# nzw0301/SimCLR

Hardware: AMD Instinct MI355X
Metric: pretrain images/sec (whole node) + CIFAR-10 linear-probe top-1, ResNet-50 (higher is better)
Workload: dtype bf16

## Files before the change

### simclr_amd/csrc/bindings.cpp

```cpp
#include <ATen/core/Tensor.h>
#include <ATen/ops/empty.h>
#include <ATen/ops/zeros.h>
#include <ATen/hip/HIPContext.h>
#include <c10/util/Exception.h>
#include <torch/library.h>

#include <algorithm>
#include <vector>

#include "kernels.h"

using at::Tensor;

namespace {

hipStream_t cur_stream() { return at::hip::getCurrentHIPStream().stream(); }

void check_dev(const Tensor& t, at::ScalarType dt, const char* name) {
  TORCH_CHECK(t.is_cuda(), name, ": expected a GPU tensor");
  TORCH_CHECK(t.scalar_type() == dt, name, ": expected dtype ", dt, " got ", t.scalar_type());
  TORCH_CHECK(t.is_contiguous(), name, ": expected a contiguous tensor");
}

const uint16_t* bf(const Tensor& t, const char* n) {
// ... 176 lines not shown
  if (f.pro_sc) {
    TORCH_CHECK(pro_seg_rows > 0 && pro_seg_rows % bm == 0 && M % pro_seg_rows == 0,
                "igemm prologue: segment rows must be a multiple of the tile rows");
    TORCH_CHECK(pro_sc->numel() >= (M / pro_seg_rows) * g.C, "igemm prologue: [S][C] size");
  }
  if (pro_d.has_value() && pro_d->defined()) {
    TORCH_CHECK(f.pro_sc, "igemm BN-backward prologue needs pro_sc (A) and pro_sh (B)");
    TORCH_CHECK(pro_d->numel() >= (M / pro_seg_rows) * g.C, "igemm prologue: d [S][C] size");
    TORCH_CHECK(A2.has_value() && A2->numel() == A.numel(), "igemm prologue: A2 must match A");
    TORCH_CHECK(epi_mode == 0 || epi_mode == 3 || epi_mode == 4,
                "igemm BN-backward prologue: epilogue 0, 3 or 4");
    TORCH_CHECK(!(igemm_variant_patch((int)variant) && epi_mode == 4),
                "igemm BN-backward prologue on a patch variant: epilogue 0 or 3");
    f.pro_d = f32(*pro_d, "pro_d");
    f.A2 = bf(*A2, "A2");
    if (pro_out.has_value() && pro_out->defined()) {
      TORCH_CHECK(igemm_variant_patch((int)variant) && (epi_mode == 0 || epi_mode == 3),
                  "igemm: the materialised BN-backward operand (pro_out) needs a patch variant "
                  "and epilogue 0 or 3");
      TORCH_CHECK(pro_out->numel() == A.numel(), "igemm: pro_out must match A");
      const char* o0 = static_cast<const char*>(pro_out->data_ptr());
      const char* o1 = o0 + pro_out->numel() * 2;
      for (const Tensor* t : {&A, &*A2, &out}) {
        const char* t0 = static_cast<const char*>(t->data_ptr());
        const char* t1 = t0 + t->numel() * t->element_size();
        TORCH_CHECK(!(o0 < t1 && t0 < o1), "igemm: pro_out must not alias A, A2 or out");
      }
      f.pro_out = bfw(*pro_out, "pro_out");
    }
  }
  if (dual) {
    TORCH_CHECK(f.pro_sc && f.pro_sh && !f.pro_d && epi_mode == 0 && !(bias.has_value() && bias->defined()),
                "igemm block-output prologue: scale/shift tables, no other fusion");
    TORCH_CHECK(A2.has_value() && A2->numel() == A.numel(), "igemm block-output prologue: residual");
    TORCH_CHECK(pro_out->numel() == A.numel(), "igemm block-output prologue: out size");
    TORCH_CHECK(pro_mask.has_value() && pro_mask->defined() && pro_mask->numel() * 8 >= A.numel(),
                "igemm block-output prologue: mask size");
    check_dev(*pro_mask, at::kByte, "pro_mask");
    TORCH_CHECK(pro_relu, "igemm block-output prologue: always applies ReLU (pro_relu required)");
    auto overlaps = [](const Tensor& a, const Tensor& b) {
      const char* a0 = static_cast<const char*>(a.data_ptr());
      const char* b0 = static_cast<const char*>(b.data_ptr());
      const char* a1 = a0 + a.numel() * a.element_size();
      const char* b1 = b0 + b.numel() * b.element_size();
      return a0 < b1 && b0 < a1;
    };
    TORCH_CHECK(!overlaps(*pro_out, A) && !overlaps(*pro_out, *A2) && !overlaps(*pro_out, out) &&
                    !overlaps(*pro_mask, A) && !overlaps(*pro_mask, *A2) && !overlaps(*pro_mask, out),
                "igemm block-output prologue: out / mask must not alias A, the residual or the "
                "conv output");
    f.A2 = bf(*A2, "A2");
    f.pro_out = bfw(*pro_out, "pro_out");
    f.pro_mask = pro_mask->data_ptr<uint8_t>();
    if (pro_rss.has_value() && pro_rss->defined()) {
      const int64_t nseg = M / pro_seg_rows;
      TORCH_CHECK(pro_rss->numel() >= 2 * nseg * g.C, "igemm block-output prologue: rss [2][S][C]");
      f.pro_rsc = f32(*pro_rss, "pro_rss");
      f.pro_rsh = f.pro_rsc + nseg * g.C;
    }
  }
  conv_igemm_nt(g, bf(A, "A"), (size_t)A.numel(), bf(B, "B"), bfw(out, "out"), optf32(bias, "bias"),
                optf32w(stats, "stats"), f, (int)variant, cur_stream());
}

int64_t igemm_bm(int64_t N) { return igemm_block_m((int)N); }
int64_t igemm_nvariants() { return igemm_num_variants(); }
int64_t igemm_vbm(int64_t v) { return igemm_variant_bm((int)v); }
int64_t igemm_vbn(int64_t v) { return igemm_variant_bn((int)v); }
bool igemm_vglds(int64_t v) { return igemm_variant_glds((int)v); }
bool igemm_gldsok(std::vector<int64_t> gv, bool pro, bool bn_bwd_pro) {
  return igemm_glds_ok(geom_from(gv), pro, bn_bwd_pro);
}
int64_t wgrad_nvariants() { return wgrad_num_variants(); }
int64_t wgrad_xlin_op(int64_t mode) { return wgrad_xlin((int)mode); }
bool wgrad_vglds(int64_t v) { return wgrad_variant_glds((int)v); }
bool igemm_vok(int64_t v, std::vector<int64_t> gv, bool pro, bool bnb, int64_t epi_mode) {
  return igemm_variant_ok((int)v, geom_from(gv), pro, bnb, (int)epi_mode);
}
bool igemm_dok(int64_t v, std::vector<int64_t> gv) { return igemm_dual_ok((int)v, geom_from(gv)); }
bool wgrad_vok(int64_t v, std::vector<int64_t> gv, bool pro, bool dpro) {
  return wgrad_variant_ok((int)v, geom_from(gv), pro, dpro);
}

int64_t wgrad_nsplit(std::vector<int64_t> gv, int64_t variant) {
  return wgrad_splits(geom_from(gv), (int)variant);
}

int64_t wgrad_ntiles(std::vector<int64_t> gv, int64_t variant) {
  return wgrad_tiles(geom_from(gv), (int)variant);
}

void wgrad(const Tensor& dY, const Tensor& X, const Tensor& partial, const Tensor& out,
           std::vector<int64_t> gv, int64_t splits, int64_t creal, double beta,
           const c10::optional<Tensor>& pro_sc, const c10::optional<Tensor>& pro_sh,
           int64_t pro_seg_rows, bool pro_relu, int64_t pro_S, int64_t variant,
           const c10::optional<Tensor>& dY2, const c10::optional<Tensor>& dp_coef,
           int64_t dp_seg_rows, int64_t dp_S) {
  const ConvGeom g = geom_from(gv);
  const int64_t M = (int64_t)g.Nb * g.OH * g.OW;
  const int64_t K = (int64_t)g.KH * g.KW * g.C;
  TORCH_CHECK(dY.numel() == M * g.N, "wgrad: dY numel mismatch");
  TORCH_CHECK(X.numel() == (int64_t)g.Nb * g.IH * g.IW * g.C, "wgrad: X numel mismatch");
  TORCH_CHECK(partial.numel() >= splits * g.N * K, "wgrad: partial too small");
  TORCH_CHECK(out.numel() == (int64_t)g.N * g.KH * g.KW * creal, "wgrad: out numel mismatch");
  TORCH_CHECK(creal <= g.C && creal > 0, "wgrad: bad creal");
  TORCH_CHECK(pro_S >= 1 && pro_S <= 2, "wgrad prologue supports at most 2 segments");
  if (variant < 0 || variant >= wgrad_num_variants()) variant = wgrad_default_variant(g.N);
  TORCH_CHECK(wgrad_variant_ok((int)variant, g, pro_sc.has_value() && pro_sc->defined(),
                               dY2.has_value() && dY2->defined()),
              "wgrad: variant ", variant, " is not admissible here: an LDS-DMA variant needs "
              "C % 64 == 0, no dY prologue, and an X prologue only on unpadded 1x1 convolutions "
              "(wgrad_pipe / wgrad_xp: none); the patch variant needs its 3x3 stride-1 geometry, "
              "N % 64 == 0 and no dY prologue");
  ConvFusion f = fusion_from(pro_sc, pro_sh, pro_seg_rows, pro_relu, pro_S, 0, c10::nullopt,
                             c10::nullopt, g.C, 0);
  if (f.pro_sc) {
    TORCH_CHECK(pro_seg_rows > 0 && (int64_t)g.Nb % pro_S == 0, "wgrad prologue geometry");
  }
  if (dY2.has_value() && dY2->defined()) {
    TORCH_CHECK(dY2->numel() == dY.numel(), "wgrad: dY2 must match dY");
    TORCH_CHECK(dp_coef.has_value() && dp_coef->numel() >= 3 * dp_S * g.N, "wgrad: dp_coef [3][S][N]");
    const int64_t iters = (M + 63) / 64;
    const int64_t ips = (iters + splits - 1) / splits;
    TORCH_CHECK(dp_seg_rows > 0 && M % dp_seg_rows == 0 && M / dp_seg_rows == dp_S &&
                    (dp_S <= 2 || dp_seg_rows % (ips * 64) == 0) && dp_seg_rows % 64 == 0,
                "wgrad dY prologue: 64-row segments, and every split inside one segment when "
                "there are more than two");
    f.dY2 = bf(*dY2, "dY2");
    f.dp_coef = f32(*dp_coef, "dp_coef");
    f.dp_seg_rows = (int)dp_seg_rows;
    f.dp_S = (int)dp_S;
  }
  conv_wgrad(g, bf(dY, "dY"), bf(X, "X"), (size_t)X.numel(), f32w(partial, "partial"), (int)splits,
             f32w(out, "out"), (int)creal, (float)beta, f, (int)variant, cur_stream());
}


void conv1x1_bwd_dual_op(const Tensor& G, const c10::optional<Tensor>& A3,
                         const c10::optional<Tensor>& coef, const Tensor& X,
                         const c10::optional<Tensor>& xss, const c10::optional<Tensor>& xmi,
                         const Tensor& Wt, const Tensor& gm,
                         const Tensor& stats, const Tensor& wpart, int64_t S, int64_t bps,
                         const c10::optional<Tensor>& Xraw, bool dual8) {
  const int64_t CI = gm.size(-1);
  const int64_t M = gm.numel() / CI;
  const int64_t CO = G.numel() / M;
  const uint16_t* xr = optbf(Xraw, "Xraw");
  TORCH_CHECK((CO == 256 && CI == 64 && xr == nullptr) || (CO == 512 && CI == 128),
              "conv1x1_bwd_dual: (Co, Ci) = (256, 64) or (512, 128); a pre-applied X (Xraw "
              "given) only with (512, 128)");
  if (xr != nullptr) TORCH_CHECK(Xraw->numel() == M * CI, "conv1x1_bwd_dual: Xraw size");
  TORCH_CHECK(G.numel() == M * CO && X.numel() == M * CI && Wt.numel() == CI * CO,
              "conv1x1_bwd_dual: operand sizes");
  TORCH_CHECK(S >= 1 && S <= 2 && bps >= 1 && M % S == 0 && (M / S) % (64 * bps) == 0,
              "conv1x1_bwd_dual: every block's rows must lie in one segment (64-row tiles)");
  const float* xs = optf32(xss, "xss");
  const float* xm = optf32(xmi, "xmi");
  TORCH_CHECK((xs == nullptr) == (xm == nullptr), "conv1x1_bwd_dual: xss and xmi together");
  TORCH_CHECK(xs != nullptr || (CO == 256 && CI == 64 && xr == nullptr),
              "conv1x1_bwd_dual: the plain form is (Co, Ci) = (256, 64) only");
  if (xs != nullptr) {
    TORCH_CHECK(xss->numel() >= 2 * S * CI && xmi->numel() >= 2 * S * CI,
                "conv1x1_bwd_dual: BN2 tables");
    TORCH_CHECK(stats.numel() >= S * bps * 2 * CI, "conv1x1_bwd_dual: stats size");
  }
  TORCH_CHECK(wpart.numel() >= S * bps * CO * CI, "conv1x1_bwd_dual: wpart size");
  TORCH_CHECK(M * CO * 2 < (int64_t(1) << 31), "conv1x1_bwd_dual: 32-bit buffer offsets");
  const uint16_t* a3 = optbf(A3, "A3");
  const float* cf = optf32(coef, "coef");
  if (a3 != nullptr) {
    TORCH_CHECK(A3->numel() == G.numel() && cf != nullptr && coef->numel() >= 3 * S * CO,
                "conv1x1_bwd_dual: lazy BN-backward needs A3 [M][Co] and coef [3][S][Co]");
  }
  conv1x1_bwd_dual(bf(G, "G"), a3, cf, bf(X, "X"), xs, xm,
                   bf(Wt, "Wt"), bfw(gm, "gm"), f32w(stats, "stats"), f32w(wpart, "wpart"),
                   (int)M, (int)CO, (int)CI, (int)S, (int)bps, cur_stream(), xr, dual8);
}

void conv1x1_bwd_dual_s2_op(const Tensor& G, const c10::optional<Tensor>& A3,
                            const c10::optional<Tensor>& coef, const Tensor& X, const Tensor& Wt,
                            const Tensor& gm, const Tensor& wpart, int64_t S, int64_t bps) {
  TORCH_CHECK(X.dim() == 4 && gm.dim() == 4, "conv1x1_bwd_dual_s2: NHWC 4-D X and gm");
  const int64_t N = X.size(0), H = X.size(1), W = X.size(2), CI = X.size(3);
  const int64_t OH = gm.size(1), OW = gm.size(2);
  TORCH_CHECK(gm.size(0) == N && gm.size(3) == CI && OH == (H + 1) / 2 && OW == (W + 1) / 2,
              "conv1x1_bwd_dual_s2: gm is the stride-2 output map");
  const int64_t Mo = N * OH * OW;
  const int64_t CO = G.numel() / Mo;
  TORCH_CHECK(CO == 512 && CI == 256 && G.numel() == Mo * CO && Wt.numel() == CI * CO,
              "conv1x1_bwd_dual_s2: (Co, Ci) = (512, 256) only");
  TORCH_CHECK(S >= 1 && S <= 2 && N % S == 0 && bps >= 1 && (Mo / S) % (64 * bps) == 0,
              "conv1x1_bwd_dual_s2: every block's rows must lie in one segment");
  TORCH_CHECK(wpart.numel() >= S * bps * CO * CI, "conv1x1_bwd_dual_s2: wpart size");
  TORCH_CHECK(Mo * CO * 2 < (int64_t(1) << 31) && X.numel() * 2 < (int64_t(1) << 31),
              "conv1x1_bwd_dual_s2: 32-bit buffer offsets");
  const uint16_t* a3 = optbf(A3, "A3");
  const float* cf = optf32(coef, "coef");
  TORCH_CHECK(a3 == nullptr && cf == nullptr,
              "conv1x1_bwd_dual_s2: dY must be materialised (no lazy BN-backward form)");
  conv1x1_bwd_dual_s2(bf(G, "G"), a3, cf, bf(X, "X"), bf(Wt, "Wt"), bfw(gm, "gm"),
                      f32w(wpart, "wpart"), (int)Mo, (int)CO, (int)CI, (int)S, (int)bps, (int)H,
                      (int)W, (int)OH, (int)OW, cur_stream());
}

void wgrad_reduce_slabs_op(const Tensor& partial, int64_t splits, const Tensor& out, double beta) {
  const int64_t n = out.numel();
  TORCH_CHECK(n % 4 == 0 && partial.numel() >= splits * n && splits >= 1,
              "wgrad_reduce_slabs: sizes");
  wgrad_reduce_slabs(f32w(partial, "partial"), (int)splits, f32w(out, "out"), (size_t)n,
                     (float)beta, cur_stream());
}

void weight_transform(const Tensor& W, const Tensor& Wt, std::vector<int64_t> p) {
  TORCH_CHECK(p.size() == 10, "weight_transform params");
  const int Co = p[0], KH = p[1], KW = p[2], Ci = p[3], KHs = p[4], KWs = p[5];
  TORCH_CHECK(W.numel() == (int64_t)Co * KH * KW * Ci, "weight_transform: W numel");
  TORCH_CHECK(Wt.numel() == (int64_t)Ci * KHs * KWs * Co, "weight_transform: Wt numel");
  for (int a = 0; a < KHs; ++a) {
    const int kh = (int)p[6] + a * (int)p[7];
    TORCH_CHECK(kh >= 0 && kh < KH, "weight_transform: kh out of range");
  }
  for (int a = 0; a < KWs; ++a) {
    const int kw = (int)p[8] + a * (int)p[9];
    TORCH_CHECK(kw >= 0 && kw < KW, "weight_transform: kw out of range");
  }
  conv_weight_transform(bf(W, "W"), bfw(Wt, "Wt"), Co, KH, KW, Ci, KHs, KWs, p[6], p[7], p[8], p[9],
                        cur_stream());
}

Tensor weight_transform_plan(const std::vector<Tensor>& Ws, const std::vector<Tensor>& Wts,
                             std::vector<int64_t> p) {
  const size_t n = Ws.size();
  TORCH_CHECK(n > 0 && Wts.size() == n && p.size() == 10 * n, "weight_transform_plan sizes");
  Tensor host = at::empty({(int64_t)(n * sizeof(WtDesc) / 8) + 1},
                          at::TensorOptions().dtype(at::kLong));
  WtDesc* d = reinterpret_cast<WtDesc*>(host.data_ptr<int64_t>());
  int blk = 0;
  for (size_t i = 0; i < n; ++i) {
    const int64_t* q = p.data() + 10 * i;
    const int Co = q[0], KH = q[1], KW = q[2], Ci = q[3], KHs = q[4], KWs = q[5];
    TORCH_CHECK(Ws[i].numel() == (int64_t)Co * KH * KW * Ci, "weight_transform_plan: W numel");
    TORCH_CHECK(Wts[i].numel() == (int64_t)Ci * KHs * KWs * Co, "weight_transform_plan: Wt numel");
    TORCH_CHECK(Ws[i].device() == Wts[0].device() && Wts[i].device() == Wts[0].device(),
                "weight_transform_plan: one device");
    for (int a = 0; a < KHs; ++a)
      TORCH_CHECK(q[6] + a * q[7] >= 0 && q[6] + a * q[7] < KH, "weight_transform_plan: kh");
    for (int a = 0; a < KWs; ++a)
      TORCH_CHECK(q[8] + a * q[9] >= 0 && q[8] + a * q[9] < KW, "weight_transform_plan: kw");
    const int nb = ((Co + 63) / 64) * ((Ci + 63) / 64) * KHs * KWs;
    d[i] = WtDesc{bf(Ws[i], "W"), bfw(Wts[i], "Wt"), Co, KH, KW, Ci, KHs, KWs, (int)q[6],
                  (int)q[7], (int)q[8], (int)q[9], blk, nb};
    blk += nb;
  }
  host.data_ptr<int64_t>()[n * sizeof(WtDesc) / 8] = blk;
  return host;
}

void weight_transform_batch(const Tensor& table, int64_t total_blocks) {
  TORCH_CHECK(table.is_cuda() && table.scalar_type() == at::kLong && table.numel() % 8 == 0 &&
                  table.numel() > 0 && total_blocks > 0,
              "weight_transform_batch: device descriptors from weight_transform_plan");
  conv_weight_transform_batch(reinterpret_cast<const WtDesc*>(table.data_ptr<int64_t>()),
                              (int)(table.numel() / 8), (int)total_blocks, cur_stream());
}

void check_rc(const Tensor& x, int64_t S, const char* n) {
  TORCH_CHECK(x.dim() >= 2, n, ": rank");
  const int64_t C = x.size(-1);
  TORCH_CHECK(C % 8 == 0, n, ": channels must be a multiple of 8");
  const int64_t CH = C / 8;
  TORCH_CHECK(CH <= 256 || CH % 256 == 0, n, ": unsupported channel count");
  TORCH_CHECK((x.numel() / C) % S == 0, n, ": rows not divisible by segments");
}

int64_t bn_blocks(int64_t R, int64_t C, int64_t S) {
  return bn_stats_blocks_per_seg((int)R, (int)C, (int)S);
}

void bn_stats(const Tensor& x, int64_t S, const Tensor& partial) {
  check_rc(x, S, "bn_stats");
  const int C = x.size(-1), R = x.numel() / C;
  const int nblk = bn_stats_blocks_per_seg(R, C, S);
  TORCH_CHECK(partial.numel() >= (int64_t)S * nblk * 2 * C, "bn_stats: partial too small");
  bn_stats_partial(bf(x, "x"), R, C, S, f32w(partial, "partial"), nullptr, cur_stream());
}

void bn_reduce(const Tensor& partial, int64_t nblk, int64_t S, int64_t C, const Tensor& stats) {
  TORCH_CHECK(partial.numel() >= S * nblk * 2 * C && stats.numel() >= 2 * S * C, "bn_reduce sizes");
  const int G = bn_reduce_groups((int)nblk);
  TORCH_CHECK(G == 1 || C % 4 == 0, "bn_reduce: C must be a multiple of 4 (float4 partial rows)");
  at::Tensor ws;
  float* wsp = nullptr;
  if (G > 1) {
    ws = at::empty({S * G * 2 * C}, stats.options());
    wsp = ws.data_ptr<float>();
  }
  bn_reduce_partials(f32(partial, "partial"), nblk, S, C, f32w(stats, "stats"), wsp, cur_stream());
}

void bn_final(const Tensor& stats, int64_t S, int64_t C, double count, double eps, double momentum,
              const c10::optional<Tensor>& rm, const c10::optional<Tensor>& rv, const Tensor& mi,
              const c10::optional<Tensor>& nbt, const c10::optional<Tensor>& gamma,
              const c10::optional<Tensor>& beta, const c10::optional<Tensor>& ss) {
  if (ss.has_value() && ss->defined()) TORCH_CHECK(ss->numel() >= 2 * S * C, "bn_finalize: ss size");
  if (gamma.has_value() && gamma->defined()) TORCH_CHECK(gamma->numel() == C, "bn_finalize: gamma");
  if (beta.has_value() && beta->defined()) TORCH_CHECK(beta->numel() == C, "bn_finalize: beta");
  TORCH_CHECK(stats.numel() >= 2 * S * C && mi.numel() >= 2 * S * C, "bn_finalize sizes");
  int64_t* nb = nullptr;
// ... 1073 lines not shown
```

### simclr_amd/csrc/conv.hip

```cpp
#include <cstring>
#include "common.h"
#include "kernels.h"

#include <type_traits>
#include <utility>

namespace {

struct IgemmArgs {
  const uint16_t* A;
  const uint16_t* B;
  uint16_t* out;
  const float* bias;
  float* stats;
  int M, N, K;
  int IH, IW, C;
  int OH, OW, KW;
  int ish, isw, dh, dw, ih0, iw0;
  int OHp, OWp, osh, osw, ooh, oow, ldo;
  int direct_out;
  uint32_t a_bytes, b_bytes;
  int nMb, nNb;
  const float* pro_sc;
  const float* pro_sh;
// ... 2515 lines not shown
#pragma unroll
    for (int j = 0; j < 8; ++j) {
      const uint32_t off = (uint32_t)(((size_t)(m0 + grow + 8 * j) * CO + gch * 8) * 2);
      G8[j] = __builtin_amdgcn_raw_buffer_load_b128(rg, off, 0, 0);
      if (lazy) A8[j] = __builtin_amdgcn_raw_buffer_load_b128(ra, off, 0, 0);
    }
#pragma unroll
    for (int j = 0; j < 2; ++j)
      X2[j] = __builtin_amdgcn_raw_buffer_load_b128(
          rx, (uint32_t)(((size_t)(m0 + xrow + 32 * j) * CI + xch * 8) * 2), 0, 0);
  };
  auto lstore = [&](int buf, const u32x4 (&G8)[8], const u32x4 (&A8)[8], const u32x4 (&X2)[2]) {
#pragma unroll
    for (int j = 0; j < 8; ++j) {
      const int r = grow + 8 * j;
      *(u32x4*)(Ds + buf * BMT * CO + r * CO + tr_swz<CO>(r, gch * 8)) =
          lazy ? bnbwd8(G8[j], A8[j], cA, cB, cD, true) : G8[j];
    }
#pragma unroll
    for (int j = 0; j < 2; ++j) {
      const int r = xrow + 32 * j;
      *(u32x4*)(Xs + buf * BMT * CI + r * CI + tr_swz<CI>(r, xch * 8)) =
          PLAIN ? X2[j] : affine_relu8(X2[j], xsc, xsh, true, true);
      if (!PLAIN) *(u32x4*)(Xr + buf * BMT * CI + r * CI + xch * 8) = X2[j];
    }
  };

  f32x4 accw[4][4];
#pragma unroll
  for (int i = 0; i < 4; ++i)
#pragma unroll
    for (int j = 0; j < 4; ++j) accw[i][j] = (f32x4){0.f, 0.f, 0.f, 0.f};
  float s1[4][4], s2[4][4];
#pragma unroll
  for (int i = 0; i < 4; ++i)
#pragma unroll
    for (int j = 0; j < 4; ++j) { s1[i][j] = 0.f; s2[i][j] = 0.f; }

  auto compute = [&](int t) {
    const int cur = t & 1;
    const uint16_t* Db = Ds + cur * BMT * CO;
    f32x4 accd[4];
#pragma unroll
    for (int fn = 0; fn < 4; ++fn) accd[fn] = (f32x4){0.f, 0.f, 0.f, 0.f};
    const int mrow = wid * 16 + li;
#pragma unroll
    for (int ks = 0; ks < CO / 32; ++ks) {
      const int lch = ks * 4 + g;
      const bf16x8 bfr = *(const bf16x8*)(Db + mrow * CO + tr_swz<CO>(mrow, lch * 8));
#pragma unroll
      for (int fn = 0; fn < 4; ++fn) {
        const int wr = fn * 16 + li;
        const bf16x8 af = *(const bf16x8*)(Ws + wr * CO + ((lch ^ (wr & 7)) * 8));
        accd[fn] = __builtin_amdgcn_mfma_f32_16x16x32_bf16(af, bfr, accd[fn], 0, 0, 0);
      }
    }
    wgrad_mma<CO, CI, 4, 1>(Db, Xs + cur * BMT * CI, accw);
    const int m = mbeg + t * BMT + mrow;
    if constexpr (PLAIN) {
#pragma unroll
      for (int fn = 0; fn < 4; ++fn) {
        const int ci = fn * 16 + 4 * g;
        const u32x2 w = {pack2bf(accd[fn][0], accd[fn][1]), pack2bf(accd[fn][2], accd[fn][3])};
        __builtin_nontemporal_store(w, (u32x2*)(p.gm + (size_t)m * CI + ci));
      }
      return;
    }
    const uint16_t* xr = Xr + cur * BMT * CI + mrow * CI;
#pragma unroll
    for (int fn = 0; fn < 4; ++fn) {
      const int ci = fn * 16 + 4 * g;
      const u32x2 yv = *(const u32x2*)(xr + ci);
      const float4 tsc = *(const float4*)(Tb + ci), tsh = *(const float4*)(Tb + CI + ci);
      const float4 tmu = *(const float4*)(Tb + 2 * CI + ci);
      const float4 tin = *(const float4*)(Tb + 3 * CI + ci);
      const float y[4] = {lo_bf(yv.x), hi_bf(yv.x), lo_bf(yv.y), hi_bf(yv.y)};
      const float sc4[4] = {tsc.x, tsc.y, tsc.z, tsc.w}, sh4[4] = {tsh.x, tsh.y, tsh.z, tsh.w};
      const float mu4[4] = {tmu.x, tmu.y, tmu.z, tmu.w}, in4[4] = {tin.x, tin.y, tin.z, tin.w};
      float gv[4];
#pragma unroll
      for (int r = 0; r < 4; ++r) {
        const float a = bf2f(f2bf(accd[fn][r]));
        gv[r] = y[r] * sc4[r] + sh4[r] > 0.f ? a : 0.f;
        s1[fn][r] += gv[r];
        s2[fn][r] += gv[r] * ((y[r] - mu4[r]) * in4[r]);
      }
      const u32x2 w = {pack2bf(gv[0], gv[1]), pack2bf(gv[2], gv[3])};
      __builtin_nontemporal_store(w, (u32x2*)(p.gm + (size_t)m * CI + ci));
    }
  };

  if (T > 0) {
    gload(0, rG[0], rA[0], rX[0]);
    lstore(0, rG[0], rA[0], rX[0]);
  }
  if (T > 1) gload(1, rG[1], rA[1], rX[1]);
  __syncthreads();
  for (int t = 0; t < T; t += 2) {
    if (t + 2 < T) gload(t + 2, rG[0], rA[0], rX[0]);
    compute(t);
    if (t + 1 < T) lstore(1, rG[1], rA[1], rX[1]);
    asm volatile("s_waitcnt lgkmcnt(0)" ::: "memory");
    __builtin_amdgcn_s_barrier();
    if (t + 1 >= T) break;
    if (t + 3 < T) gload(t + 3, rG[1], rA[1], rX[1]);
    compute(t + 1);
    if (t + 2 < T) lstore(0, rG[0], rA[0], rX[0]);
    asm volatile("s_waitcnt lgkmcnt(0)" ::: "memory");
    __builtin_amdgcn_s_barrier();
  }
  __syncthreads();
  float* wp = p.wpart + (size_t)blk * CO * CI;
#pragma unroll
  for (int fm = 0; fm < 4; ++fm)
#pragma unroll
    for (int fn = 0; fn < 4; ++fn)
#pragma unroll
      for (int i = 0; i < 4; ++i)
        wp[(size_t)(wid * 64 + fm * 16 + g * 4 + i) * CI + fn * 16 + li] = accw[fm][fn][i];
  if (PLAIN) return;
#pragma unroll
  for (int off = 1; off < 16; off <<= 1)
#pragma unroll
    for (int fn = 0; fn < 4; ++fn)
#pragma unroll
      for (int r = 0; r < 4; ++r) {
        s1[fn][r] += __shfl_xor(s1[fn][r], off, 64);
        s2[fn][r] += __shfl_xor(s2[fn][r], off, 64);
      }
  if (li == 0) {
#pragma unroll
    for (int fn = 0; fn < 4; ++fn)
#pragma unroll
      for (int r = 0; r < 4; ++r) {
        const int ci = fn * 16 + 4 * g + r;
        red[(wid * CI + ci) * 2 + 0] = s1[fn][r];
        red[(wid * CI + ci) * 2 + 1] = s2[fn][r];
      }
  }
  __syncthreads();
  if (tid < CI) {
    float a = 0.f, b = 0.f;
#pragma unroll
    for (int w = 0; w < 4; ++w) {
      a += red[(w * CI + tid) * 2 + 0];
      b += red[(w * CI + tid) * 2 + 1];
    }
    p.stats[((size_t)blk * 2 + 0) * CI + tid] = a;
    p.stats[((size_t)blk * 2 + 1) * CI + tid] = b;
  }
}

template <int CO, int CIT, bool LAZY, bool XPRE, bool PLAIN = false, bool XS2 = false,
          int BMT = 32>
__global__ __launch_bounds__(512, 1) void conv1x1_bwd_dual_w(Dual1x1Args p) {
  constexpr int CI = 64;
  constexpr int NH = CIT / CI;
  constexpr int NT = 512;
  constexpr int RG = BMT / 16;
  constexpr int CQ = 8 / RG;
  constexpr int CW = CI / CQ;
  constexpr int NF = CW / 16;
  static_assert((CO == 512 && BMT == 32) || (CO == 256 && BMT == 64), "dual tile mappings");
  static_assert(CIT % CI == 0 && NF >= 1, "dual tile mapping");
  static_assert(!XS2 || PLAIN, "the strided X form is the plain downsample form");
  static_assert(!XPRE || BMT * (CI / 8) == 256, "XPRE: half the threads load the raw operand");
  extern __shared__ __attribute__((aligned(16))) char smem[];
  uint16_t* Ds = (uint16_t*)smem;
  uint16_t* Xs = Ds + 2 * BMT * CO;
  constexpr int XRS = CI + 8;
  uint16_t* Xr = Xs + 2 * BMT * CI;
  uint16_t* Ws = Xr + 2 * BMT * XRS;
  float* red = (float*)(Ws + CI * CO);
  float* Tb = red + RG * CI * 2;
  float* Cf = Tb + 4 * CI;

  const int tid = threadIdx.x, lane = tid & 63;
  const int wid = __builtin_amdgcn_readfirstlane(tid >> 6);
  const int g = lane >> 4, li = lane & 15;
  const int rh = wid % RG, cq = wid / RG;
  const int lb = xcd_remap(blockIdx.x, gridDim.x);
  const int half = lb % NH;
  const int blk = lb / NH;
  const int c0 = half * CI;
  const int seg = blk / p.bps;
  const int mbeg = seg * p.seg_rows + (blk - seg * p.bps) * p.tiles_per_block * BMT;
  const int T = p.tiles_per_block;

  const __amdgpu_buffer_rsrc_t rg = buf_rsrc(p.G, p.g_bytes);
  const __amdgpu_buffer_rsrc_t ra = buf_rsrc(LAZY ? p.A3 : p.G, p.g_bytes);
  const __amdgpu_buffer_rsrc_t rx = buf_rsrc((XPRE && wid >= 4) ? p.Xraw : p.X, p.x_bytes);

  for (int c = tid; c < CI * CO / 8; c += NT) {
    const int row = c / (CO / 8), ch = c % (CO / 8);
    *(u32x4*)(Ws + row * CO + ((ch ^ (row & 15)) * 8)) =
        *(const u32x4*)(p.Wt + ((size_t)(c0 + row) * CO + ch * 8));
  }
  for (int i = tid; i < (PLAIN ? 0 : 4 * CI); i += NT) {
    const int k = i / CI, c = i % CI;
    Tb[i] = (k < 2 ? p.xss : p.xmi)[((k & 1) * p.S + seg) * CIT + c0 + c];
  }
  if (LAZY)
    for (int i = tid; i < 3 * CO; i += NT) {
      const int k = i / CO, c = i % CO;
      Cf[i] = p.coef[(k * p.S + seg) * CO + c];
    }
  constexpr int GCH = CO / 8, XCH = CI / 8;
  constexpr int GR = NT / GCH;
  constexpr int GJ = BMT / GR;
  constexpr int XT = BMT * XCH;
  static_assert(XT == 256 || XT == 512, "X chunk mapping");
  const int gch = tid % GCH, grow = tid / GCH;
  const int xt = tid % XT, xch = xt % XCH, xrow = xt / XCH;
  const bool xload = XT == 512 || (XPRE && !PLAIN) || wid < 4;
  const bool xown = XT == 512 || wid < 4;

  u32x4 rG[2][GJ], rA[2][GJ], rX[2];
  uint32_t xs_n = 0, xs_oh = 0, xs_ow = 0;
  if (XS2) {
    const uint32_t m = (uint32_t)(mbeg + xrow), ohw = (uint32_t)(p.xOH * p.xOW);
    xs_n = m / ohw;
    const uint32_t rem = m - xs_n * ohw;
    xs_oh = rem / (uint32_t)p.xOW;
    xs_ow = rem - xs_oh * (uint32_t)p.xOW;
  }
  auto gload = [&](int t, u32x4 (&G8)[GJ], u32x4 (&A8)[GJ], u32x4& X1) {
    const int m0 = mbeg + t * BMT;
#pragma unroll
    for (int j = 0; j < GJ; ++j) {
      const uint32_t off = (uint32_t)(((size_t)(m0 + grow + GR * j) * CO + gch * 8) * 2);
      G8[j] = __builtin_amdgcn_raw_buffer_load_b128(rg, off, 0, 0);
      if (LAZY) A8[j] = __builtin_amdgcn_raw_buffer_load_b128(ra, off, 0, 0);
    }
    if (xload) {
      uint32_t xr_ = (uint32_t)(m0 + xrow);
      if constexpr (XS2) {
        xr_ = (xs_n * (uint32_t)p.xH + 2u * xs_oh) * (uint32_t)p.xW + 2u * xs_ow;
        xs_ow += BMT;
        while (xs_ow >= (uint32_t)p.xOW) { xs_ow -= (uint32_t)p.xOW; ++xs_oh; }
        while (xs_oh >= (uint32_t)p.xOH) { xs_oh -= (uint32_t)p.xOH; ++xs_n; }
      }
      X1 = __builtin_amdgcn_raw_buffer_load_b128(
          rx, (xr_ * (uint32_t)CIT + (uint32_t)(c0 + xch * 8)) * 2u, 0, 0);
    }
  };
  auto lstore = [&](int buf, const u32x4 (&G8)[GJ], const u32x4 (&A8)[GJ], const u32x4& X1) {
#pragma unroll
    for (int j = 0; j < GJ; ++j) {
      const int r = grow + GR * j;
      u32x4 v = G8[j];
      if (LAZY) v = bnbwd8(G8[j], A8[j], Cf + gch * 8, Cf + CO + gch * 8, Cf + 2 * CO + gch * 8,
                           true);
      *(u32x4*)(Ds + buf * BMT * CO + r * CO + tr_swz<CO>(r, gch * 8)) = v;
    }
    if (xown) {
      *(u32x4*)(Xs + buf * BMT * CI + xrow * CI + tr_swz<CI>(xrow, xch * 8)) =
          (XPRE || PLAIN) ? X1 : affine_relu8(X1, Tb + xch * 8, Tb + CI + xch * 8, true, true);
      if (!XPRE && !PLAIN) *(u32x4*)(Xr + buf * BMT * XRS + xrow * XRS + xch * 8) = X1;
    } else if (XPRE && !PLAIN) {
      *(u32x4*)(Xr + buf * BMT * XRS + xrow * XRS + xch * 8) = X1;
    }
  };

  f32x4 accw[CO / 8 / 16][CI / 16];
#pragma unroll
  for (int i = 0; i < CO / 8 / 16; ++i)
#pragma unroll
    for (int j = 0; j < CI / 16; ++j) accw[i][j] = (f32x4){0.f, 0.f, 0.f, 0.f};
  float s1[NF][4], s2[NF][4];
#pragma unroll
  for (int fn = 0; fn < NF; ++fn)
#pragma unroll
    for (int r = 0; r < 4; ++r) { s1[fn][r] = 0.f; s2[fn][r] = 0.f; }

  auto compute = [&](int t) {
    const int cur = t & 1;
    const uint16_t* Db = Ds + cur * BMT * CO;
    f32x4 accd[NF];
#pragma unroll
    for (int fn = 0; fn < NF; ++fn) accd[fn] = (f32x4){0.f, 0.f, 0.f, 0.f};
    const int mrow = rh * 16 + li;
#pragma unroll 4
    for (int ks = 0; ks < CO / 32; ++ks) {
      const int lch = ks * 4 + g;
      const bf16x8 bfr = *(const bf16x8*)(Db + mrow * CO + tr_swz<CO>(mrow, lch * 8));
#pragma unroll
      for (int fn = 0; fn < NF; ++fn) {
        const int wr = cq * CW + fn * 16 + li;
        const bf16x8 af = *(const bf16x8*)(Ws + wr * CO + ((lch ^ (wr & 15)) * 8));
        accd[fn] = __builtin_amdgcn_mfma_f32_16x16x32_bf16(af, bfr, accd[fn], 0, 0, 0);
      }
    }
    wgrad_mma<CO, CI, 8, 1, BMT / 32>(Db, Xs + cur * BMT * CI, accw);
    const int m = mbeg + t * BMT + mrow;
#pragma unroll
    for (int fn = 0; fn < NF; ++fn) {
    const int ci = cq * CW + fn * 16 + 4 * g;
    if constexpr (PLAIN) {
      const u32x2 w = {pack2bf(accd[fn][0], accd[fn][1]), pack2bf(accd[fn][2], accd[fn][3])};
      __builtin_nontemporal_store(w, (u32x2*)(p.gm + (size_t)m * CIT + c0 + ci));
    } else {
    const uint16_t* xr = Xr + cur * BMT * XRS + mrow * XRS;
    const u32x2 yv = *(const u32x2*)(xr + ci);
    const float4 tsc = *(const float4*)(Tb + ci), tsh = *(const float4*)(Tb + CI + ci);
    const float4 tmu = *(const float4*)(Tb + 2 * CI + ci);
    const float4 tin = *(const float4*)(Tb + 3 * CI + ci);
    const float y[4] = {lo_bf(yv.x), hi_bf(yv.x), lo_bf(yv.y), hi_bf(yv.y)};
    const float sc4[4] = {tsc.x, tsc.y, tsc.z, tsc.w}, sh4[4] = {tsh.x, tsh.y, tsh.z, tsh.w};
    const float mu4[4] = {tmu.x, tmu.y, tmu.z, tmu.w}, in4[4] = {tin.x, tin.y, tin.z, tin.w};
    float gv[4];
#pragma unroll
    for (int r = 0; r < 4; ++r) {
      const float a = bf2f(f2bf(accd[fn][r]));
      gv[r] = y[r] * sc4[r] + sh4[r] > 0.f ? a : 0.f;
      s1[fn][r] += gv[r];
      s2[fn][r] += gv[r] * ((y[r] - mu4[r]) * in4[r]);
    }
    const u32x2 w = {pack2bf(gv[0], gv[1]), pack2bf(gv[2], gv[3])};
    __builtin_nontemporal_store(w, (u32x2*)(p.gm + (size_t)m * CIT + c0 + ci));
    }
    }
  };

  __syncthreads();
  if (T > 0) {
    gload(0, rG[0], rA[0], rX[0]);
    lstore(0, rG[0], rA[0], rX[0]);
  }
  if (T > 1) gload(1, rG[1], rA[1], rX[1]);
  __syncthreads();
  for (int t = 0; t < T; t += 2) {
    if (t + 2 < T) gload(t + 2, rG[0], rA[0], rX[0]);
    if constexpr (PLAIN) __builtin_amdgcn_sched_barrier(0);
    compute(t);
    if constexpr (PLAIN) __builtin_amdgcn_sched_barrier(0);
    if (t + 1 < T) lstore(1, rG[1], rA[1], rX[1]);
    asm volatile("s_waitcnt lgkmcnt(0)" ::: "memory");
    __builtin_amdgcn_s_barrier();
    if (t + 1 >= T) break;
    if (t + 3 < T) gload(t + 3, rG[1], rA[1], rX[1]);
    if constexpr (PLAIN) __builtin_amdgcn_sched_barrier(0);
    compute(t + 1);
    if constexpr (PLAIN) __builtin_amdgcn_sched_barrier(0);
    if (t + 2 < T) lstore(0, rG[0], rA[0], rX[0]);
    asm volatile("s_waitcnt lgkmcnt(0)" ::: "memory");
    __builtin_amdgcn_s_barrier();
  }
  __syncthreads();
  float* wp = p.wpart + (size_t)blk * CO * CIT;
#pragma unroll
  for (int fm = 0; fm < CO / 8 / 16; ++fm)
#pragma unroll
    for (int fn = 0; fn < CI / 16; ++fn)
#pragma unroll
      for (int i = 0; i < 4; ++i)
        wp[(size_t)(wid * (CO / 8) + fm * 16 + g * 4 + i) * CIT + c0 + fn * 16 + li] =
            accw[fm][fn][i];
  if (PLAIN) return;
#pragma unroll
  for (int off = 1; off < 16; off <<= 1)
#pragma unroll
    for (int fn = 0; fn < NF; ++fn)
#pragma unroll
      for (int r = 0; r < 4; ++r) {
        s1[fn][r] += __shfl_xor(s1[fn][r], off, 64);
        s2[fn][r] += __shfl_xor(s2[fn][r], off, 64);
      }
  if (li == 0) {
#pragma unroll
    for (int fn = 0; fn < NF; ++fn)
#pragma unroll
      for (int r = 0; r < 4; ++r) {
        const int ci = cq * CW + fn * 16 + 4 * g + r;
        red[(rh * CI + ci) * 2 + 0] = s1[fn][r];
        red[(rh * CI + ci) * 2 + 1] = s2[fn][r];
      }
  }
  __syncthreads();
  if (tid < CI) {
    float a = 0.f, b = 0.f;
#pragma unroll
    for (int q = 0; q < RG; ++q) {
      a += red[(q * CI + tid) * 2 + 0];
      b += red[(q * CI + tid) * 2 + 1];
    }
    p.stats[((size_t)blk * 2 + 0) * CIT + c0 + tid] = a;
    p.stats[((size_t)blk * 2 + 1) * CIT + c0 + tid] = b;
  }
}

}

void conv_weight_transform_batch(const WtDesc* d, int n, int total_blocks, hipStream_t s) {
  hipLaunchKernelGGL(weight_transform_batch, dim3(total_blocks), dim3(256), 0, s, d, n);
  HIP_CHECK_LAUNCH();
}

int igemm_num_variants() { return kNumIgemm; }
int igemm_variant_bm(int v) { return IG_VARIANTS[v].bm; }
int igemm_variant_bn(int v) { return IG_VARIANTS[v].bn; }
int igemm_default_variant(int N) { return N <= 64 ? 1 : 0; }
bool igemm_variant_glds(int v) { return v >= 0 && v < kNumIgemm && IG_VARIANTS[v].fam != IG_NT; }
bool igemm_variant_patch(int v) {
  return v >= 0 && v < kNumIgemm && IG_VARIANTS[v].fam == IG_PATCH;
}
bool igemm_glds_ok(const ConvGeom& g, bool pro, bool bn_bwd_pro) {
  if (g.C % 64 != 0) return false;
  return !(pro || bn_bwd_pro) || (g.KH == 1 && g.KW == 1 && g.ih0 == 0 && g.iw0 == 0);
}
static bool direct_out(const ConvGeom& g) {
  return g.osh == 1 && g.osw == 1 && g.ooh == 0 && g.oow == 0 && g.OHp == g.OH && g.OWp == g.OW;
}
bool igemm_patch_ok(const ConvGeom& g) {
  return g.KH == 3 && g.KW == 3 && g.ish == 1 && g.isw == 1 && g.dh == 1 && g.dw == 1 &&
         g.ih0 == -1 && g.iw0 == -1 && g.OH == g.IH && g.OW == g.IW &&
         (g.OW == 16 || g.OW == 32) && (g.C == 64 || g.C == 128) && direct_out(g);
}
static bool glds_doubled_fits(const IgemmVariant& r, const ConvGeom& g, int words) {
  const size_t lds = igemm_glds_pro_offset(r.bm, r.bn, r.threads(), g.C > 64 ? 2 : 1, 2) +
                     (size_t)4 * words * g.C;
  return lds <= 160 * 1024;
}
bool igemm_dual_ok(int v, const ConvGeom& g) {
  if (v < 0 || v >= kNumIgemm) return false;
  const IgemmVariant& r = IG_VARIANTS[v];
  if (!r.fuses(3, 0) || !igemm_glds_ok(g, true, false)) return false;
  if (!(direct_out(g) && g.ish == 1 && g.isw == 1 && g.OH == g.IH && g.OW == g.IW)) return false;
  if ((g.Nb * g.OH * g.OW) % r.bm) return false;
  return glds_doubled_fits(r, g, 4);
}

bool igemm_variant_ok(int v, const ConvGeom& g, bool pro, bool bn_bwd_pro, int epi_mode) {
  if (v < 0 || v >= kNumIgemm) return false;
  const IgemmVariant& r = IG_VARIANTS[v];
  const bool bwd4 = bn_bwd_pro && (epi_mode & 255) == 4 && r.fam == IG_GLDS;
  if (!r.fuses(igemm_pro_code(pro, bn_bwd_pro, false), bwd4 ? 4 : 0)) return false;
  switch (r.fam) {
    case IG_NT: return true;
    case IG_PATCH: {
      if (!igemm_patch_ok(g)) return false;
      if (!bn_bwd_pro) return true;
      const int TR = 256 / g.OW, PP = (TR + 2) * (g.OW + 2), NT = r.threads();
      return (PP * (g.C / 8) + NT - 1) / NT <= kPatchBnbChunks;
    }
    case IG_GLDS:
      return (!bn_bwd_pro || glds_doubled_fits(r, g, 3)) && igemm_glds_ok(g, pro, bn_bwd_pro);
  }
  return false;
}
int igemm_block_m(int N) { return igemm_variant_bm(igemm_default_variant(N)); }

void conv_igemm_nt(const ConvGeom& g, const uint16_t* A, size_t a_elems, const uint16_t* B,
                   uint16_t* out, const float* bias, float* stats, const ConvFusion& f,
                   int variant, hipStream_t s) {
  IgemmArgs a{};
  a.A = A; a.B = B; a.out = out; a.bias = bias; a.stats = stats;
  a.M = g.Nb * g.OH * g.OW; a.N = g.N; a.K = g.KH * g.KW * g.C;
  a.IH = g.IH; a.IW = g.IW; a.C = g.C;
  a.OH = g.OH; a.OW = g.OW; a.KW = g.KW;
  a.ish = g.ish; a.isw = g.isw; a.dh = g.dh; a.dw = g.dw; a.ih0 = g.ih0; a.iw0 = g.iw0;
  a.OHp = g.OHp; a.OWp = g.OWp; a.osh = g.osh; a.osw = g.osw; a.ooh = g.ooh; a.oow = g.oow;
  a.ldo = g.ldo;
  a.direct_out = direct_out(g) ? 1 : 0;
  a.a_bytes = (uint32_t)(a_elems * 2);
  a.b_bytes = (uint32_t)((size_t)a.N * a.K * 2);
  a.pro_sc = f.pro_sc; a.pro_sh = f.pro_sh; a.pro_seg_rows = f.pro_seg_rows > 0 ? f.pro_seg_rows : a.M;
  a.pro_relu = f.pro_relu;
  a.pro_d = f.pro_d; a.A2 = f.A2;
  a.pro_rsc = f.pro_rsc; a.pro_rsh = f.pro_rsh; a.pro_out = f.pro_out; a.pro_mask = f.pro_mask;
  a.epi_mode = f.epi_mode; a.epi_a_sub = f.epi_a_sub; a.epi_a = f.epi_a; a.epi_b = f.epi_b; a.epi_c = f.epi_c;
  a.epi_mask = f.epi_mask;
  a.epi_c2 = f.epi_c2; a.epi_mi2 = f.epi_mi2; a.stats2 = f.stats2;
  a.epi_ss = f.epi_ss; a.epi_mi = f.epi_mi; a.epi_S = f.epi_S > 0 ? f.epi_S : 1;
  a.seg_rows = f.seg_rows; a.stats_seg_blocks = f.stats_seg_blocks; a.stats_base = f.stats_base;
  if (variant < 0 || variant >= igemm_num_variants()) variant = igemm_default_variant(g.N);
  const bool dual = a.pro_out != nullptr && a.pro_d == nullptr;
  if (dual ? !igemm_dual_ok(variant, g)
           : !igemm_variant_ok(variant, g, a.pro_sc != nullptr, a.pro_d != nullptr, a.epi_mode)) {
    fprintf(stderr, "igemm: variant %d: unsupported geometry / fusion\n", variant);
    abort();
  }
  IG_VARIANTS[variant].launch(a, s);
}


int wgrad_num_variants() { return kNumWgrad; }
int wgrad_xlin(int mode) { return xlin_mode(mode); }
int wgrad_default_variant(int N) { return N <= 64 ? 1 : 0; }
bool wgrad_variant_glds(int v) { return v >= 0 && v < kNumWgrad && WG_VARIANTS[v].lds_dma(); }
int wgrad_variant_area(int v) { return WG_VARIANTS[v].bco * WG_VARIANTS[v].bkk; }
bool wgrad_variant_ok(int v, const ConvGeom& g, bool pro, bool dy_pro) {
  if (v < 0 || v >= kNumWgrad) return false;
  const WgradVariant& r = WG_VARIANTS[v];
  if ((pro && !r.x_pro()) || (dy_pro && !r.dy_pro())) return false;
  if (r.fam == WG_PATCH) return g.N % 64 == 0 && igemm_patch_ok(g);
  return !r.lds_dma() || igemm_glds_ok(g, pro, false);
}

int wgrad_tiles(const ConvGeom& g, int variant) {
  if (variant < 0 || variant >= kNumWgrad) variant = wgrad_default_variant(g.N);
  const WgradVariant& r = WG_VARIANTS[variant];
  return ((g.N + r.bco - 1) / r.bco) * r.k_tiles(g.C, g.KH * g.KW * g.C);
}

int wgrad_splits(const ConvGeom& g, int variant) {
  if (variant < 0 || variant >= kNumWgrad) variant = wgrad_default_variant(g.N);
  const WgradVariant& r = WG_VARIANTS[variant];
  const int tiles = wgrad_tiles(g, variant);
  const int iters = r.iters(g.Nb * g.OH * g.OW);
  static const int pct = [] {
    const char* e = getenv("SIMCLR_WGRAD_TARGET_PCT");
    const int v = e ? atoi(e) : 80;
    return v > 0 ? v : 100;
  }();
  const int target = std::max(1, r.target * pct / 100);
  const int splits = (target + tiles - 1) / tiles;
  return std::max(1, std::min(splits, iters / r.min_iters()));
}

struct SlabsLeft { int count, stride; };
static SlabsLeft reduce_slabs_l1(float* partial, int splits, size_t n4, hipStream_t s) {
  constexpr int GROUP = 16;
  if (splits <= 2 * GROUP) return {splits, 1};
  const int G = (splits + GROUP - 1) / GROUP;
  const int bx = (int)std::min<size_t>((n4 + 255) / 256, 1024);
  hipLaunchKernelGGL(wgrad_reduce_l1, dim3(bx, G), dim3(256), 0, s, (float4*)partial, splits,
                     GROUP, n4);
  HIP_CHECK_LAUNCH();
  return {G, GROUP};
}
static void reduce_slabs(float* partial, int splits, float* out, size_t n4, float beta, bool vec4,
                         hipStream_t s) {
  if (vec4 && reduce_cols_ok(n4, splits)) {
    hipLaunchKernelGGL(wgrad_reduce_cols, dim3((unsigned)((n4 + RC_COLS - 1) / RC_COLS)),
                       dim3(256), 0, s, (const float4*)partial, (float4*)out, splits, n4, beta);
    HIP_CHECK_LAUNCH();
    return;
  }
  const SlabsLeft left = vec4 ? reduce_slabs_l1(partial, splits, n4, s) : SlabsLeft{splits, 1};
  const int blocks = (int)std::min<size_t>((n4 + 255) / 256, 8192);
  hipLaunchKernelGGL(wgrad_reduce_vec4, dim3(blocks), dim3(256), 0, s, (const float4*)partial,
                     (float4*)out, left.count, left.stride, n4, beta);
  HIP_CHECK_LAUNCH();
}

void conv_wgrad(const ConvGeom& g, const uint16_t* dY, const uint16_t* X, size_t x_elems,
                float* partial, int splits, float* out, int Creal, float beta,
                const ConvFusion& f, int variant, hipStream_t s) {
  WgradArgs a{};
  a.dY = dY; a.X = X; a.partial = partial;
  a.M = g.Nb * g.OH * g.OW; a.N = g.N; a.K = g.KH * g.KW * g.C;
  a.IH = g.IH; a.IW = g.IW; a.C = g.C;
  a.OH = g.OH; a.OW = g.OW; a.KW = g.KW;
  a.ish = g.ish; a.isw = g.isw; a.dh = g.dh; a.dw = g.dw; a.ih0 = g.ih0; a.iw0 = g.iw0;
  a.dy_bytes = (uint32_t)((size_t)a.M * a.N * 2);
  a.x_bytes = (uint32_t)(x_elems * 2);
  if (variant < 0 || variant >= kNumWgrad) variant = wgrad_default_variant(g.N);
  const WgradVariant& r = WG_VARIANTS[variant];
  const int iters = r.iters(a.M);
  a.splits = splits;
  a.iters_per_split = (iters + splits - 1) / splits;
  a.pro_sc = f.pro_sc; a.pro_sh = f.pro_sh;
  a.pro_seg_rows = f.pro_seg_rows > 0 ? f.pro_seg_rows : a.M;
  a.pro_relu = f.pro_relu; a.pro_S = f.pro_S > 0 ? f.pro_S : 1;
  a.dY2 = f.dY2; a.dp_coef = f.dp_coef; a.dp_seg_rows = f.dp_seg_rows > 0 ? f.dp_seg_rows : a.M;
  a.dp_S = f.dp_S > 0 ? f.dp_S : 1;
  a.slab_stride = (size_t)a.N * a.K;
  static const int slab_exp = [] {
    const char* e = getenv("SIMCLR_EXPERIMENT_WGRAD_SLABS");
    if (!e) return 0;
    if (!strcmp(e, "noreduce")) return 1;
    if (!strcmp(e, "alias")) return 2;
    return 0;
  }();
  if (slab_exp == 2) a.slab_stride = 0;
  if (!wgrad_variant_ok(variant, g, a.pro_sc != nullptr, a.dY2 != nullptr)) {
    fprintf(stderr, "wgrad: variant %d: unsupported geometry / prologue\n", variant);
    abort();
  }
  r.launch(a, s);
  const int K = a.K;
  if (splits == 1 && partial == out && Creal == g.C && beta == 0.f) return;
  if (slab_exp != 0) return;
  const size_t n4 = (size_t)a.N * K / 4;
  const bool vec4 = (a.N * K) % 4 == 0;
  if (Creal == g.C) {
    reduce_slabs(partial, splits, out, n4, beta, vec4, s);
    return;
  }
  const SlabsLeft left = vec4 ? reduce_slabs_l1(partial, splits, n4, s) : SlabsLeft{splits, 1};
  const size_t total = (size_t)a.N * (K / g.C) * Creal;
  const int cb = (int)std::min<size_t>((total + 255) / 256, 4096);
  if (left.count > 1 && vec4) {
    const int blocks = (int)std::min<size_t>((n4 + 255) / 256, 8192);
    hipLaunchKernelGGL(wgrad_reduce_vec4_inplace, dim3(blocks), dim3(256), 0, s,
                       (float4*)partial, left.count, left.stride, n4);
    HIP_CHECK_LAUNCH();
    hipLaunchKernelGGL(wgrad_reduce, dim3(cb), dim3(256), 0, s, partial, out, 1, 1, a.N, K, g.C,
                       Creal, beta);
  } else {
    hipLaunchKernelGGL(wgrad_reduce, dim3(cb), dim3(256), 0, s, partial, out, left.count,
                       left.stride, a.N, K, g.C, Creal, beta);
  }
  HIP_CHECK_LAUNCH();
}

void conv_weight_transform(const uint16_t* W, uint16_t* Wt, int Co, int KH, int KW, int Ci,
                           int KHs, int KWs, int kh0, int sh, int kw0, int sw, hipStream_t s) {
  const size_t total = (size_t)Ci * KHs * KWs * Co;
  int blocks = (int)((total + 255) / 256);
  if (blocks > 4096) blocks = 4096;
  hipLaunchKernelGGL(weight_transform, dim3(blocks), dim3(256), 0, s, W, Wt, Co, KH, KW, Ci, KHs,
                     KWs, kh0, sh, kw0, sw);
  HIP_CHECK_LAUNCH();
}

size_t conv1x1_bwd_dual_lds() {
  return (size_t)2 * 64 * 256 * 2 + 2 * (size_t)2 * 64 * 64 * 2 + (size_t)64 * 256 * 2 +
         (size_t)4 * 64 * 2 * 4 + (size_t)4 * 64 * 4;
}

size_t conv1x1_bwd_dual_w_lds(int CO, int BMT = 32) {
  return (size_t)2 * BMT * CO * 2 + (size_t)2 * BMT * (64 + 72) * 2 + (size_t)64 * CO * 2 +
         (size_t)(BMT / 16) * 64 * 2 * 4 + (size_t)4 * 64 * 4 + (size_t)3 * CO * 4;
}

void conv1x1_bwd_dual(const uint16_t* G, const uint16_t* A3, const float* coef, const uint16_t* X,
                      const float* xss, const float* xmi, const uint16_t* Wt, uint16_t* gm,
                      float* stats, float* wpart, int M, int CO, int CI, int S, int bps,
                      hipStream_t s, const uint16_t* Xraw, bool dual8) {
  Dual1x1Args a{};
  a.G = G; a.A3 = A3; a.coef = coef; a.X = X; a.xss = xss; a.xmi = xmi; a.Wt = Wt; a.gm = gm;
  a.stats = stats; a.wpart = wpart;
  a.M = M; a.S = S; a.seg_rows = M / S; a.bps = bps;
  a.tiles_per_block = a.seg_rows / 64 / bps;
  a.g_bytes = (uint32_t)((size_t)M * CO * 2);
  a.x_bytes = (uint32_t)((size_t)M * CI * 2);
  a.Xraw = Xraw;
  a.x_pre = Xraw != nullptr;
  const size_t lds = conv1x1_bwd_dual_lds();
  if (CO == 512 && CI == 128) {
    a.tiles_per_block = a.seg_rows / 32 / bps;
    const dim3 grid(S * bps * 2), blk(512);
    const size_t wl = conv1x1_bwd_dual_w_lds(512);
    if (A3 != nullptr && Xraw != nullptr)
      hipLaunchKernelGGL((conv1x1_bwd_dual_w<512, 128, true, true>), grid, blk, wl, s, a);
    else if (A3 != nullptr)
      hipLaunchKernelGGL((conv1x1_bwd_dual_w<512, 128, true, false>), grid, blk, wl, s, a);
    else if (Xraw != nullptr)
      hipLaunchKernelGGL((conv1x1_bwd_dual_w<512, 128, false, true>), grid, blk, wl, s, a);
    else
      hipLaunchKernelGGL((conv1x1_bwd_dual_w<512, 128, false, false>), grid, blk, wl, s, a);
  } else if (CO == 256 && CI == 64 && Xraw == nullptr && dual8) {
    const dim3 grid(S * bps), blk(512);
    const size_t wl = conv1x1_bwd_dual_w_lds(256, 64);
    if (xss == nullptr && A3 != nullptr)
      hipLaunchKernelGGL((conv1x1_bwd_dual_w<256, 64, true, false, true, false, 64>), grid, blk,
                         wl, s, a);
    else if (xss == nullptr)
      hipLaunchKernelGGL((conv1x1_bwd_dual_w<256, 64, false, false, true, false, 64>), grid, blk,
                         wl, s, a);
    else if (A3 != nullptr)
      hipLaunchKernelGGL((conv1x1_bwd_dual_w<256, 64, true, false, false, false, 64>), grid, blk,
                         wl, s, a);
    else
      hipLaunchKernelGGL((conv1x1_bwd_dual_w<256, 64, false, false, false, false, 64>), grid,
                         blk, wl, s, a);
  } else if (CO == 256 && CI == 64 && xss == nullptr) {
    hipLaunchKernelGGL((conv1x1_bwd_dual<256, 64, true>), dim3(S * bps), dim3(256), lds, s, a);
  } else if (CO == 256 && CI == 64 && Xraw == nullptr) {
    hipLaunchKernelGGL((conv1x1_bwd_dual<256, 64>), dim3(S * bps), dim3(256), lds, s, a);
  } else {
    fprintf(stderr, "conv1x1_bwd_dual: unsupported Co=%d Ci=%d\n", CO, CI);
    abort();
  }
  HIP_CHECK_LAUNCH();
}

void conv1x1_bwd_dual_s2(const uint16_t* G, const uint16_t* A3, const float* coef,
                         const uint16_t* X, const uint16_t* Wt, uint16_t* gm, float* wpart,
                         int Mo, int CO, int CI, int S, int bps, int H, int W, int OH, int OW,
                         hipStream_t s) {
  Dual1x1Args a{};
  a.G = G; a.A3 = A3; a.coef = coef; a.X = X; a.Wt = Wt; a.gm = gm; a.wpart = wpart;
  a.M = Mo; a.S = S; a.seg_rows = Mo / S; a.bps = bps;
  a.tiles_per_block = a.seg_rows / 32 / bps;
  a.g_bytes = (uint32_t)((size_t)Mo * CO * 2);
  a.x_bytes = (uint32_t)((size_t)(Mo / (OH * OW)) * H * W * CI * 2);
  a.xH = H; a.xW = W; a.xOH = OH; a.xOW = OW;
  if (CO != 512 || CI != 256) {
    fprintf(stderr, "conv1x1_bwd_dual_s2: unsupported Co=%d Ci=%d\n", CO, CI);
    abort();
  }
  const dim3 grid(S * bps * (CI / 64)), blk(512);
  const size_t wl = conv1x1_bwd_dual_w_lds(512);
  hipLaunchKernelGGL((conv1x1_bwd_dual_w<512, 256, false, false, true, true>), grid, blk, wl, s,
                     a);
  HIP_CHECK_LAUNCH();
}

void wgrad_reduce_slabs(float* partial, int splits, float* out, size_t n, float beta,
                        hipStream_t s) {
  reduce_slabs(partial, splits, out, n / 4, beta, true, s);
}
```

Before: 24830.

## Add optional three-deep register prefetch to dual 1x1 conv backward kernel

Adds a DEPTH template parameter so the dual 1x1 backward weight/data kernel can keep three operand tiles in flight in registers instead of two. The loop is restructured into a phase lambda, and out-of-range loads are made safe by setting the buffer offset high bit so they fall outside the buffer and need no branch. The depth-3 variants are used only when SIMCLR_DUAL_DEPTH=3 is set; the default path is still depth 2 but now runs the branchless loop. Deeper prefetch raises register pressure and may cause spills.

```diff
diff --git a/simclr_amd/csrc/bindings.cpp b/simclr_amd/csrc/bindings.cpp
--- a/simclr_amd/csrc/bindings.cpp
+++ b/simclr_amd/csrc/bindings.cpp
@@ -352,8 +352,10 @@
   if (xr != nullptr) TORCH_CHECK(Xraw->numel() == M * CI, "conv1x1_bwd_dual: Xraw size");
   TORCH_CHECK(G.numel() == M * CO && X.numel() == M * CI && Wt.numel() == CI * CO,
               "conv1x1_bwd_dual: operand sizes");
-  TORCH_CHECK(S >= 1 && S <= 2 && bps >= 1 && M % S == 0 && (M / S) % (64 * bps) == 0,
-              "conv1x1_bwd_dual: every block's rows must lie in one segment (64-row tiles)");
+  const int64_t tile = CO == 512 ? 32 : 64;
+  TORCH_CHECK(S >= 1 && S <= 2 && bps >= 1 && M % S == 0 && (M / S) % (tile * bps) == 0,
+              "conv1x1_bwd_dual: every block's rows must lie in one segment (whole 64-row "
+              "tiles, 32-row in the wide form)");
   const float* xs = optf32(xss, "xss");
   const float* xm = optf32(xmi, "xmi");
   TORCH_CHECK((xs == nullptr) == (xm == nullptr), "conv1x1_bwd_dual: xss and xmi together");
diff --git a/simclr_amd/csrc/conv.hip b/simclr_amd/csrc/conv.hip
--- a/simclr_amd/csrc/conv.hip
+++ b/simclr_amd/csrc/conv.hip
@@ -2691,8 +2691,9 @@
 }
 
 template <int CO, int CIT, bool LAZY, bool XPRE, bool PLAIN = false, bool XS2 = false,
-          int BMT = 32>
+          int BMT = 32, int DEPTH = 2>
 __global__ __launch_bounds__(512, 1) void conv1x1_bwd_dual_w(Dual1x1Args p) {
+  static_assert(DEPTH == 2 || DEPTH == 3, "operand tiles in flight (register sets)");
   constexpr int CI = 64;
   constexpr int NH = CIT / CI;
   constexpr int NT = 512;
@@ -2754,7 +2755,7 @@
   const bool xload = XT == 512 || (XPRE && !PLAIN) || wid < 4;
   const bool xown = XT == 512 || wid < 4;
 
-  u32x4 rG[2][GJ], rA[2][GJ], rX[2];
+  u32x4 rG[DEPTH][GJ], rA[DEPTH][GJ], rX[DEPTH];
   uint32_t xs_n = 0, xs_oh = 0, xs_ow = 0;
   if (XS2) {
     const uint32_t m = (uint32_t)(mbeg + xrow), ohw = (uint32_t)(p.xOH * p.xOW);
@@ -2765,9 +2766,11 @@
   }
   auto gload = [&](int t, u32x4 (&G8)[GJ], u32x4 (&A8)[GJ], u32x4& X1) {
     const int m0 = mbeg + t * BMT;
+    const uint32_t dead = t < T ? 0u : 0x80000000u;
 #pragma unroll
     for (int j = 0; j < GJ; ++j) {
-      const uint32_t off = (uint32_t)(((size_t)(m0 + grow + GR * j) * CO + gch * 8) * 2);
+      const uint32_t off =
+          (uint32_t)(((size_t)(m0 + grow + GR * j) * CO + gch * 8) * 2) | dead;
       G8[j] = __builtin_amdgcn_raw_buffer_load_b128(rg, off, 0, 0);
       if (LAZY) A8[j] = __builtin_amdgcn_raw_buffer_load_b128(ra, off, 0, 0);
     }
@@ -2780,7 +2783,7 @@
         while (xs_oh >= (uint32_t)p.xOH) { xs_oh -= (uint32_t)p.xOH; ++xs_n; }
       }
       X1 = __builtin_amdgcn_raw_buffer_load_b128(
-          rx, (xr_ * (uint32_t)CIT + (uint32_t)(c0 + xch * 8)) * 2u, 0, 0);
+          rx, ((xr_ * (uint32_t)CIT + (uint32_t)(c0 + xch * 8)) * 2u) | dead, 0, 0);
     }
   };
   auto lstore = [&](int buf, const u32x4 (&G8)[GJ], const u32x4 (&A8)[GJ], const u32x4& X1) {
@@ -2862,28 +2865,27 @@
   };
 
   __syncthreads();
-  if (T > 0) {
-    gload(0, rG[0], rA[0], rX[0]);
-    lstore(0, rG[0], rA[0], rX[0]);
-  }
-  if (T > 1) gload(1, rG[1], rA[1], rX[1]);
+  gload(0, rG[0], rA[0], rX[0]);
+  lstore(0, rG[0], rA[0], rX[0]);
+#pragma unroll
+  for (int k = 1; k < DEPTH; ++k) gload(k, rG[k], rA[k], rX[k]);
   __syncthreads();
-  for (int t = 0; t < T; t += 2) {
-    if (t + 2 < T) gload(t + 2, rG[0], rA[0], rX[0]);
+  auto phase = [&](int t, u32x4 (&Gf)[GJ], u32x4 (&Af)[GJ], u32x4& Xf, const u32x4 (&Gn)[GJ],
+                   const u32x4 (&An)[GJ], const u32x4& Xn) {
+    gload(t + DEPTH, Gf, Af, Xf);
     if constexpr (PLAIN) __builtin_amdgcn_sched_barrier(0);
     compute(t);
     if constexpr (PLAIN) __builtin_amdgcn_sched_barrier(0);
-    if (t + 1 < T) lstore(1, rG[1], rA[1], rX[1]);
+    lstore((t + 1) & 1, Gn, An, Xn);
     asm volatile("s_waitcnt lgkmcnt(0)" ::: "memory");
     __builtin_amdgcn_s_barrier();
-    if (t + 1 >= T) break;
-    if (t + 3 < T) gload(t + 3, rG[1], rA[1], rX[1]);
-    if constexpr (PLAIN) __builtin_amdgcn_sched_barrier(0);
-    compute(t + 1);
-    if constexpr (PLAIN) __builtin_amdgcn_sched_barrier(0);
-    if (t + 2 < T) lstore(0, rG[0], rA[0], rX[0]);
-    asm volatile("s_waitcnt lgkmcnt(0)" ::: "memory");
-    __builtin_amdgcn_s_barrier();
+    return t + 1 >= T;
+  };
+  for (int t = 0; t < T; t += DEPTH) {
+    if (phase(t, rG[0], rA[0], rX[0], rG[1], rA[1], rX[1])) break;
+    if (phase(t + 1, rG[1], rA[1], rX[1], rG[2 % DEPTH], rA[2 % DEPTH], rX[2 % DEPTH])) break;
+    if constexpr (DEPTH == 3)
+      if (phase(t + 2, rG[2 % DEPTH], rA[2 % DEPTH], rX[2 % DEPTH], rG[0], rA[0], rX[0])) break;
   }
   __syncthreads();
   float* wp = p.wpart + (size_t)blk * CO * CIT;
@@ -3164,10 +3166,16 @@
          (size_t)(BMT / 16) * 64 * 2 * 4 + (size_t)4 * 64 * 4 + (size_t)3 * CO * 4;
 }
 
+static bool dual_depth3() {
+  const char* e = getenv("SIMCLR_DUAL_DEPTH");
+  return e != nullptr && atoi(e) == 3;
+}
+
 void conv1x1_bwd_dual(const uint16_t* G, const uint16_t* A3, const float* coef, const uint16_t* X,
                       const float* xss, const float* xmi, const uint16_t* Wt, uint16_t* gm,
                       float* stats, float* wpart, int M, int CO, int CI, int S, int bps,
                       hipStream_t s, const uint16_t* Xraw, bool dual8) {
+  const bool d3 = dual_depth3();
   Dual1x1Args a{};
   a.G = G; a.A3 = A3; a.coef = coef; a.X = X; a.xss = xss; a.xmi = xmi; a.Wt = Wt; a.gm = gm;
   a.stats = stats; a.wpart = wpart;
@@ -3188,12 +3196,18 @@
       hipLaunchKernelGGL((conv1x1_bwd_dual_w<512, 128, true, false>), grid, blk, wl, s, a);
     else if (Xraw != nullptr)
       hipLaunchKernelGGL((conv1x1_bwd_dual_w<512, 128, false, true>), grid, blk, wl, s, a);
+    else if (d3)
+      hipLaunchKernelGGL((conv1x1_bwd_dual_w<512, 128, false, false, false, false, 32, 3>), grid,
+                         blk, wl, s, a);
     else
       hipLaunchKernelGGL((conv1x1_bwd_dual_w<512, 128, false, false>), grid, blk, wl, s, a);
   } else if (CO == 256 && CI == 64 && Xraw == nullptr && dual8) {
     const dim3 grid(S * bps), blk(512);
     const size_t wl = conv1x1_bwd_dual_w_lds(256, 64);
-    if (xss == nullptr && A3 != nullptr)
+    if (xss == nullptr && A3 != nullptr && d3)
+      hipLaunchKernelGGL((conv1x1_bwd_dual_w<256, 64, true, false, true, false, 64, 3>), grid,
+                         blk, wl, s, a);
+    else if (xss == nullptr && A3 != nullptr)
       hipLaunchKernelGGL((conv1x1_bwd_dual_w<256, 64, true, false, true, false, 64>), grid, blk,
                          wl, s, a);
     else if (xss == nullptr)
@@ -3202,6 +3216,9 @@
     else if (A3 != nullptr)
       hipLaunchKernelGGL((conv1x1_bwd_dual_w<256, 64, true, false, false, false, 64>), grid, blk,
                          wl, s, a);
+    else if (d3)
+      hipLaunchKernelGGL((conv1x1_bwd_dual_w<256, 64, false, false, false, false, 64, 3>), grid,
+                         blk, wl, s, a);
     else
       hipLaunchKernelGGL((conv1x1_bwd_dual_w<256, 64, false, false, false, false, 64>), grid,
                          blk, wl, s, a);
```

Result: no change. 24820 (median of 2 runs) (-0.0%).
